# hukaixuan19970627/yolov5_obb

Hardware: AMD Instinct MI355X
Metric: val.py img/s (hot path: non_max_suppression_obb, bs16) + NMS ms/img @100k cand, DOTAv1.5 1024^2, 1/2/4/8 GPU (higher is better)
Workload: dtype f16; 1 GPU; DOTAv1.5 1024^2 bs16 (BASELINE metric; configs[1] thresholds): yolov5 OBB head output (16,64512,201) fp16, 4 distinct tensors rotated (cold: 1.66 GB working set) -> non_max_suppression_obb (conf .25, iou .45, multi_label, max_det 1500), val.py --task speed hot path = dt[2] of val.py; global_batch=16, anchors_per_image=64512, nc=16, detections_per_batch=3734, parallelism=dp1 (images sharded, no data-path collective)

## Files before the change

### include/obb_hip.h

```cpp
#ifndef OBB_HIP_H
#define OBB_HIP_H

#include <stddef.h>
#include <stdint.h>

#ifdef __cplusplus
extern "C" {
#endif

#define OBB_OK 0
#define OBB_ERR_BAD_ARG (-1)
#define OBB_ERR_WORKSPACE (-2)
#define OBB_ERR_LAUNCH (-3)
#define OBB_ERR_INTERNAL (-4)
#define OBB_ERR_NO_DEVICE (-5)

#define OBB_DTYPE_F32 0
#define OBB_DTYPE_F16 1
#define OBB_DTYPE_BF16 3

#define OBB_NMS_DROP_SMALL 1

const char* obb_version(void);
int obb_device_info(int* cu_count, int* wave_size, char* arch_name, int arch_name_len);
int obb_nms_set_max_grid(int max_workgroups);

#define OBB_PROF_STAGES 8
int obb_profile_enable(int on);
int obb_profile_collect(double* ms_sum_host, int64_t* count_host, int n_stages);



size_t obb_nms_workspace_bytes(int64_t n, int64_t nseg, int kind);

int obb_nms_rotated_f32(const float* dets5, const float* scores, int64_t n, float iou_thr, int flags, int64_t max_keep,
                        int64_t* keep_out, int64_t* num_keep, void* ws, size_t ws_bytes, void* stream);

int obb_nms_rotated_f64(const double* dets5, const double* scores, int64_t n, float iou_thr, int flags, int64_t max_keep,
                        int64_t* keep_out, int64_t* num_keep, void* ws, size_t ws_bytes, void* stream);

int obb_nms_poly_f32(const float* polys, int64_t row_stride, int64_t n, float iou_thr, int64_t max_keep, int64_t* keep_out,
                     int64_t* num_keep, void* ws, size_t ws_bytes, void* stream);

int obb_merge_nms_poly_f64(const double* dets9, int64_t n, const int32_t* order, const int32_t* seg_off, int64_t nseg,
// ... 197 lines not shown
```

### yolov5_obb_amd/_lib.py

```python
import ctypes as C
import os
import threading

import torch

_HERE = os.path.dirname(os.path.abspath(__file__))
LIB_PATH = os.environ.get("OBB_HIP_LIB") or os.path.join(_HERE, "libobb_hip.so")

OBB_OK = 0
OBB_NMS_DROP_SMALL = 1
_ERR = {-1: "bad argument", -2: "workspace missing or too small", -3: "kernel launch failed",
        -4: "internal error", -5: "no usable HIP device"}

_lib = None
_lock = threading.RLock()

_vp, _i64, _i32, _f32, _sz = C.c_void_p, C.c_int64, C.c_int, C.c_float, C.c_size_t

SIGNATURES = {
    "obb_version": (C.c_char_p, []),
    "obb_device_info": (_i32, [C.POINTER(_i32), C.POINTER(_i32), C.c_char_p, _i32]),
    "obb_nms_set_max_grid": (_i32, [_i32]),
    "obb_profile_enable": (_i32, [_i32]),
    "obb_profile_collect": (_i32, [_vp, _vp, _i32]),
    "obb_nms_workspace_bytes": (_sz, [_i64, _i64, _i32]),
    "obb_nms_rotated_f32": (_i32, [_vp, _vp, _i64, _f32, _i32, _i64, _vp, _vp, _vp, _sz, _vp]),
    "obb_nms_rotated_f64": (_i32, [_vp, _vp, _i64, _f32, _i32, _i64, _vp, _vp, _vp, _sz, _vp]),
    "obb_nms_poly_f32": (_i32, [_vp, _i64, _i64, _f32, _i64, _vp, _vp, _vp, _sz, _vp]),
    "obb_merge_nms_poly_f64": (_i32, [_vp, _i64, _vp, _vp, _i64, C.c_double, _vp, _vp, _vp, _sz, _vp]),
    "obb_merge_nms_poly_all_f64": (_i32, [_vp, _i64, _vp, _vp, _i64, C.c_double, _vp, _vp, _vp, _sz, _vp]),
    "obb_merge_nms_hbb_f64": (_i32, [_vp, _i64, _i64, _vp, _vp, _i64, C.c_double, _vp, _vp, _vp, _sz, _vp]),
    "obb_task1_parse_tiles": (_i64, [_vp, _i64, _i64, _vp, _vp, _vp, _vp, _vp, _vp]),
    "obb_task1_format_rows": (_i64, [_vp, _vp, _vp, _vp, _vp, _i64, _vp, _i64]),
    "obb_task1_parse_dets": (_i64, [_vp, _i64, _i64, _vp, _vp, _vp, _vp]),
    "obb_task1_parse_gt": (_i64, [_vp, _i64, _i64, _vp, _vp, _vp, _vp]),
    "obb_eval_best_gt_f64": (_i32, [_vp, _vp, _i64, _vp, _vp, _i64, _vp, _vp, _vp]),
    "obb_eval_best_gt_hbb_f64": (_i32, [_vp, _i64, _vp, _i64, _vp, _vp, _i64, _vp, _vp, _vp]),
    "obb_nms_obb_workspace_bytes": (_sz, [_i64, _i64, _i64, _i32]),
    "obb_non_max_suppression_obb": (_i32, [_vp, _i32, _i64, _i64, _i64, _f32, _f32, _vp, _i32, _i32, _i32, _i64, _i64, _f32,
# ... 265 lines not shown
```

### yolov5_obb_amd/csrc/nms.hip

```cpp
#include <hip/hip_runtime.h>
#include <cstring>
#include <stdint.h>
#include <stdlib.h>
#include <stdio.h>
#include <string.h>
#include <hip/hip_fp16.h>
#include "launch_once.h"
#include "obb_device.h"
#include "nms_core.h"
#include "nms_mk.h"
#include "obb_hip.h"
#include "psrs_sort.h"
#include "nms_small.h"
#include "segsort.h"
#include "ws_layout.h"
#include "nms_plan.h"

namespace obb {

enum { PROF_DECODE = 0, PROF_SEGSORT, PROF_PREP, PROF_STEPS, PROF_GATHER, PROF_NMS_SORT, PROF_NMS_PREP, PROF_NMS_STEPS, PROF_N };
struct ProfState {
  int on = 0;
  static constexpr int kMax = 8192;
  hipEvent_t ev0[kMax], ev1[kMax];
// ... 957 lines not shown
}

int obb_profile_collect(double* ms_sum, int64_t* count, int n_stages) {
  for (int i = 0; i < n_stages; i++) { ms_sum[i] = 0.0; count[i] = 0; }
  for (int k = 0; k < g_prof.used; k++) {
    float ms = 0.f;
    if (hipEventSynchronize(g_prof.ev1[k]) != hipSuccess) return OBB_ERR_INTERNAL;
    if (hipEventElapsedTime(&ms, g_prof.ev0[k], g_prof.ev1[k]) != hipSuccess) return OBB_ERR_INTERNAL;
    const int id = g_prof.id[k];
    if (id < n_stages) { ms_sum[id] += ms; count[id]++; }
  }
  g_prof.used = 0;
  return OBB_OK;
}

int obb_nms_set_max_grid(int max_workgroups) {
  g_max_grid = max_workgroups > 0 ? max_workgroups : 0;
  return OBB_OK;
}

const char* obb_version(void) { return "obb_hip 0.2 (gfx950)"; }

int obb_device_info(int* cu_count, int* wave_size, char* arch_name, int arch_name_len) {
  int dev = 0;
  if (hipGetDevice(&dev) != hipSuccess) return OBB_ERR_NO_DEVICE;
  hipDeviceProp_t p;
  if (hipGetDeviceProperties(&p, dev) != hipSuccess) return OBB_ERR_NO_DEVICE;
  if (cu_count) *cu_count = p.multiProcessorCount;
  if (wave_size) *wave_size = p.warpSize;
  if (arch_name && arch_name_len > 0) { strncpy(arch_name, p.gcnArchName, arch_name_len - 1); arch_name[arch_name_len - 1] = 0; }
// ... 32 lines not shown
```

### yolov5_obb_amd/csrc/nms_plan.h

```cpp
#pragma once
#include <stddef.h>
#include <stdint.h>
#include <stdlib.h>

#include "nms_limits.h"
#include "ws_layout.h"

namespace obb {

enum FbWord {
  kFbSteps = 0,
  kFbKept = 1,
  kFbSlabs = 2,
  kFbEnqueued = 3,
  kFbTicksPersist = 4,
  kFbTicksMk = 5,
  kFbKeptPersist = 6,
  kFbKeptMk = 7,
  kFbWords = 8
};
struct FbSnapshot { int w[kFbWords]; };
static inline FbSnapshot fb_snapshot(const int* words) {
  FbSnapshot s;
  for (int i = 0; i < kFbWords; i++) s.w[i] = *(const volatile int*)(words + i);
  return s;
}

static inline int env_mk(const char* e) { return e ? atoi(e) : 2; }
static inline int env_mk_xlds(const char* e) { return (e && (e[0] == '0' || e[0] == '1')) ? e[0] - '0' : -1; }
static inline int env_small_helpers(const char* e) { const int v = (e && *e) ? atoi(e) : -1; return v > kSmallHelpMax ? kSmallHelpMax : v; }
static inline int env_self_sort(const char* e) { return (e && *e >= '0' && *e <= '2') ? *e - '0' : 2; }
static inline int env_mk_steps(const char* e) { return e ? atoi(e) : 0; }
static inline int env_mk_pend(const char* e) { const int v = e ? atoi(e) : 0; return (v > 0 && v < kMkPend1) ? v : kMkPend1; }
static inline int env_phase_prof(const char* e) { return (e && atoi(e)) ? 1 : 0; }
static inline int env_poly_strict(const char* e) { const int v = e ? atoi(e) : 0; return v == 1 ? 1 : (v >= 2 ? 0 : 3); }

struct NmsEnv {
  int mk;
  int mk_xlds;
  int small_helpers;
  int self_sort;
  int mk_steps;
  int mk_pend;
  int phase_prof;
  int quad_skip;
};
static inline NmsEnv nms_env() {
  static const NmsEnv process = [] {
    NmsEnv e{};
    e.mk_steps = env_mk_steps(getenv("OBB_NMS_MK_STEPS")); e.mk_pend = env_mk_pend(getenv("OBB_NMS_MK_PEND"));
    e.phase_prof = env_phase_prof(getenv("OBB_NMS_PHASE_PROF")); e.quad_skip = env_poly_strict(getenv("OBB_NMS_POLY_STRICT"));
    return e;
  }();
  NmsEnv e = process;
  e.mk = env_mk(getenv("OBB_NMS_MK")); e.mk_xlds = env_mk_xlds(getenv("OBB_NMS_MK_XLDS"));
  e.small_helpers = env_small_helpers(getenv("OBB_NMS_SMALL_HELPERS")); e.self_sort = env_self_sort(getenv("OBB_NMS_SELF_SORT"));
  return e;
}

static inline int nms_window(long long max_keep) {
  if (max_keep <= 0) return 0;
  long long w = 4 * max_keep;
  if (w < 8192) w = 8192;
  if (w > (1 << 30)) w = 1 << 30;
  return (int)((w + 63) / 64 * 64);
}
static inline int nms_grid(int64_t nseg, int64_t n_slots, int cap_first_, int cus) {
  int64_t nb = (n_slots + 511) / 512;
  {
    const int64_t per_seg = (n_slots + nseg - 1) / nseg;
    const int64_t c = per_seg < cap_first_ ? per_seg : cap_first_;
// ... 81 lines not shown
struct SmallHelpBlocks { int *work, *seg_np, *seg_ticket; unsigned long long *part_main, *part_help; };
static inline SmallHelpBlocks small_help_layout(WsCursor& w, int helpers, int64_t nseg, int64_t n_pos) {
  SmallHelpBlocks b;
  b.work = w.take<int>((size_t)helpers);
  b.seg_np = w.take<int>((size_t)nseg); b.seg_ticket = w.take<int>((size_t)nseg);
  b.part_main = w.take<unsigned long long>((size_t)n_pos * kSmallWords);
  b.part_help = w.take<unsigned long long>((size_t)helpers * kSmallMax * kSmallWords);
  return b;
}
static inline size_t small_help_bytes(int helpers, int64_t nseg, int64_t n_pos) {
  WsCursor w(nullptr);
  small_help_layout(w, helpers, nseg, n_pos);
  return w.total();
}

struct ObbPlanIn {
  int64_t bs, A;
  int nc, agnostic, multi_label;
  float iou_thres, max_wh;
  int64_t n_extra;
  int64_t cap_img;
  int64_t max_nms, max_det;
  int64_t expected_cand;
  int out_packed;
  int hw_cus, cus;
  long long ecap;
  size_t sort_tmp_bytes;
  size_t ps_scratch_bytes;
};
struct ObbPlan {
  int ncs;
  int class_ok;
  int multi_label;
  int64_t expected_cand, seg_hint;
  int small_hint;
  int lds_sort;
  int small_nms;
  int self_sort;
  int helpers;
  int fused_out;
  int rows_per_thread;
  int parts;
  int plan_nb, plan_chunk;
  int64_t max_seg;
  unsigned radix_mask;
  int psrs;
  unsigned gparts;
  int window;
  int zero_bar;
  int zero_alive;
};

static inline ObbPlan plan_nms_obb(const ObbPlanIn& in, const NmsEnv& env) {
  ObbPlan p{};
  const int64_t bs = in.bs, cap_img = in.cap_img;
  p.seg_hint = (in.expected_cand >> 32) & 0x1fffffff;
  p.small_hint = ((in.expected_cand >> 62) & 1) != 0;
  p.expected_cand = in.expected_cand & 0xffffffffll;
  p.ncs = in.agnostic ? 1 : in.nc;
  const int64_t nseg = bs * p.ncs;
  p.class_ok = (!in.agnostic && in.nc > 1 && in.A + in.n_extra < (1ll << 24) && in.iou_thres >= 0.f && in.max_wh > 0.f) ? 1 : 0;
  p.multi_label = (in.multi_label && in.nc > 1) ? 1 : 0;
  p.lds_sort = p.expected_cand > 0 && p.expected_cand <= kSortLdsHint;
  p.rows_per_thread = (bs * in.A >= 4LL * kDecThreads * 480) ? 4 : (bs * in.A >= 2LL * kDecThreads * 480) ? 2 : 1;
  p.max_seg = (in.max_nms > 0 && in.max_nms < cap_img) ? in.max_nms : cap_img;
// ... 16 lines not shown
    if (!p.self_sort) p.parts = (p.class_ok && p.ncs >= 8) ? 4 : 1;
  } else {
    int tb = 0;
    while ((1ll << tb) < in.A * in.nc + in.n_extra + 1) tb++;
    unsigned mask = 0xF0u;
    for (int d = 0; d < 4; d++) if (tb > d * 8) mask |= 1u << d;
    if (p.class_ok) mask = 0xFFu;
    p.radix_mask = mask;
    p.psrs = bs == 1 && cap_img <= kPsMaxN && in.sort_tmp_bytes >= in.ps_scratch_bytes;
  }
  p.fused_out = p.small_nms && !in.out_packed;
  if (!p.fused_out)
    p.gparts = p.expected_cand <= 2048 ? 1u : (unsigned)((p.expected_cand + 1023) / 1024 > 16 ? 16 : (p.expected_cand + 1023) / 1024);
  p.zero_bar = (!p.small_nms || !p.fused_out) ? 1 : 0;
  p.zero_alive = (p.lds_sort && !p.self_sort) ? 1 : 0;
  return p;
}

}
```

### yolov5_obb_amd/csrc/nms_small.h

```cpp
#pragma once
#include "nms_limits.h"

namespace obb {

#ifdef OBB_SMALL_TRACE
__device__ unsigned long long g_small_trace[2048 * 16];
__device__ unsigned long long g_small_trace_tail[2048 * 4];
__device__ unsigned long long g_small_trace2[2048 * 8];
#define STRACE(kind, ...) do { if (threadIdx.x == 0 && blockIdx.x < 2048) { const unsigned long long v_[] = {__VA_ARGS__}; unsigned long long* o_ = g_small_trace + blockIdx.x * 16; o_[0] = (kind); for (int z_ = 0; z_ < (int)(sizeof(v_) / 8) && z_ < 15; z_++) o_[1 + z_] = v_[z_]; } } while (0)
#endif
constexpr int kSmallThreads = 512;
constexpr int kSmallWaves = kSmallThreads / 64;

struct SmallArgs {
  const float4* rec;
  const u64* alive;
  const int* seg_begin;
  const int* seg_end;
  int* keep_cnt;
  int64_t* keep_out;
  int* too_big;
  float thr;
  int max_keep;
  const unsigned long long* keys_sorted;
// ... 6 lines not shown
  int helpers;
  const int* help_cnt;
  const int* work;
  const int* seg_np;
  int* seg_ticket;
  u64* part_main;
  u64* part_help;
  const unsigned long long* keys_in;
  const float4* cand;
  const int* cnt;
  const int* tiny;
  long long cap_img, max_nms, A;
  int nc;
  float class_offset;
  int* seg_max;
};
struct SmallFromSort { static constexpr bool kSelf = false; };
constexpr int kSmallClipWaves = 4;
constexpr int kSmallSplit1 = 128;
__host__ __device__ __forceinline__ int small_parts(int n) {
  return n <= kSmallSplit1 ? 1 : (n <= 192 ? 2 : (n <= 256 ? 4 : (n <= 320 ? 6 : 8)));
}
struct SmallNoTail {
  struct Args {};
  static __device__ __forceinline__ void run(const SmallArgs&, const Args&, unsigned char*, int) {}
};

template <class G>
__device__ __attribute__((noinline)) int small_quick(const float4* ra, const float4* rb, float thr) {
  return G::classify_quick(ra, rb, thr, true);
}
// ... 24 lines not shown
  uint32_t q0[128], q1[128], q2[128];
};

template <class G, class FRONT>
__device__ __forceinline__ int small_segment(const SmallArgs& a, unsigned char* s_raw) {
  __shared__ int s_next, s_nkept, s_qcnt[kSmallWaves], s_qhead[kSmallWaves], s_qcnt2[kSmallWaves], s_last;
  __shared__ uint32_t s_kept[kSmallMax];
  __shared__ unsigned long long s_pk[kSmallMax];
  __shared__ uint32_t s_pv[kSmallMax];
  float4* s_rec = reinterpret_cast<float4*>(s_raw);
  u64* s_mask = reinterpret_cast<u64*>(s_rec + (size_t)kSmallMax * G::RECQ);
  u64* s_alive = s_mask + (size_t)kSmallMax * kSmallWords;
  SmallWave<G>* s_wave = reinterpret_cast<SmallWave<G>*>(s_alive + 8);
  const int tid = threadIdx.x, lane = tid & 63, wv = tid >> 6;
  int seg = (int)blockIdx.x - a.helpers, part = 0, np = 1, hbase = 0;
  if (seg < 0) {
    const int h = (int)blockIdx.x;
    if (h >= *a.help_cnt) {
#ifdef OBB_SMALL_TRACE
      STRACE(1ull, (unsigned long long)wall_clock64());
#endif
      return -1;
    }
    const int e = a.work[h];
    if (e < 0) return -1;
    seg = e & 0xffffff; part = e >> 24;
  }
  if (a.helpers > 0) { const int v = a.seg_np[seg]; if ((v & 255) > 1) { np = v & 255; hbase = v >> 8; } }
#ifdef OBB_SMALL_TRACE
  unsigned long long tt[8]; int ti_ = 0, nd0 = 0, nd1 = 0, nd2 = 0, nit = 0;
  unsigned long long acc_d0 = 0, acc_d1 = 0, acc_d2 = 0, acc_draw = 0, acc_l0 = 0, acc_l1 = 0, acc_l2 = 0;
#define SSTAMP() do { tt[ti_++] = wall_clock64(); } while (0)
#else
#define SSTAMP() do {} while (0)
#endif
  SSTAMP();
  int sb, n, md_self = 0;
  if constexpr (FRONT::kSelf) {
    const int r = FRONT::template load<G>(a, seg, reinterpret_cast<float4*>(s_raw),
                                          reinterpret_cast<u64*>(reinterpret_cast<float4*>(s_raw) + (size_t)kSmallMax * G::RECQ), s_pk, s_pv, &s_next);
    n = r & 0xffff; md_self = r >> 16;
    sb = (int)((long long)(seg / a.ncs) * a.cap_img) + (seg % a.ncs) * kSmallMax;
    if (n <= 0 || n > kSmallMax) {
      if (tid == 0) { stg_agent(a.keep_cnt + seg, 0); if (n > kSmallMax) atomicMax(a.too_big, n); }
      return seg;
    }
  } else {
    sb = a.seg_begin[seg]; n = a.seg_end[seg] - sb;
    if (n <= 0) return part == 0 ? seg : -1;
    if (n > kSmallMax) { if (tid == 0 && part == 0) atomicMax(a.too_big, n); return part == 0 ? seg : -1; }
  }
  const bool pub = a.pub_key != nullptr;
  if constexpr (!FRONT::kSelf) {
    for (int t = tid; t < n * G::RECQ; t += kSmallThreads) s_rec[t] = a.rec[(size_t)sb * G::RECQ + t];
    for (int t = tid; t < n * kSmallWords; t += kSmallThreads) s_mask[t] = 0ull;
    if (pub)
      for (int t = tid; t < n; t += kSmallThreads) { s_pk[t] = a.keys_sorted[(size_t)sb + t]; s_pv[t] = a.vals_sorted[(size_t)sb + t]; }
    if (tid < kSmallWords) {
      const int w0 = (sb >> 6) + tid, sh = sb & 63;
      u64 v = a.alive[w0] >> sh;
// ... 171 lines not shown
          Q.head = (Q.head + took) & 127; Q.count -= took;
        }
        if (busy) {
          if (stage == 0) { Q1.push(res == 3, e); Q2.push(res == 2, e); }
          else if (stage == 1) Q2.push(res == 2, e);
          wave_sync();
        }
        __syncthreads();
      }
    }
  }
  SSTAMP();
  __syncthreads();
  if (np > 1) {
    auto part_buf = [&](int p) -> u64* {
      return p == 0 ? a.part_main + (size_t)sb * kSmallWords : a.part_help + (size_t)(hbase + p - 1) * kSmallMax * kSmallWords;
    };
    u64* mine = part_buf(part);
    for (int t = tid; t < n * kSmallWords; t += kSmallThreads) stg_agent(mine + t, s_mask[t]);
    asm volatile("s_waitcnt vmcnt(0)" ::: "memory");
    __syncthreads();
    if (tid == 0) s_last = __hip_atomic_fetch_add(a.seg_ticket + seg, 1, __ATOMIC_RELAXED, __HIP_MEMORY_SCOPE_AGENT) == np - 1 ? 1 : 0;
    __syncthreads();
    if (!s_last) {
#ifdef OBB_SMALL_TRACE
      STRACE(2ull, (unsigned long long)seg | ((unsigned long long)part << 24) | ((unsigned long long)np << 28), (unsigned long long)n, 0ull, tt[0], tt[1], tt[2], tt[3], (unsigned long long)wall_clock64(), 0ull, 0ull, (unsigned long long)nit, (unsigned long long)nd0, (unsigned long long)nd1, (unsigned long long)nd2);
#endif
      return -1;
    }
    for (int p = 0; p < np; p++) {
      if (p == part) continue;
      const u64* src = part_buf(p);
      for (int t = tid; t < n * kSmallWords; t += kSmallThreads) { const u64 v = ldg_agent(src + t); if (v) s_mask[t] |= v; }
    }
    __syncthreads();
  }
  SSTAMP();
// ... 62 lines not shown
```

### yolov5_obb_amd/csrc/nmsobb_impl.h

```cpp
#pragma once
#include "dtype_device.h"
#include "obb_device.h"
#include "segsort.h"
#include "nms_plan.h"

namespace obb {

struct ClassMask { unsigned long long w[4]; int all; };

template <typename T> __device__ __forceinline__ float mul_in_dtype(float a, float b);
template <> __device__ __forceinline__ float mul_in_dtype<float>(float a, float b) { return a * b; }
template <> __device__ __forceinline__ float mul_in_dtype<__half>(float a, float b) { return __half2float(__float2half_rn(a * b)); }
template <> __device__ __forceinline__ float mul_in_dtype<bf16_t>(float a, float b) { return round_to_dtype<bf16_t>(a * b); }
template <typename T> __device__ __forceinline__ float thr_in_dtype(float t);
template <> __device__ __forceinline__ float thr_in_dtype<float>(float t) { return t; }
template <> __device__ __forceinline__ float thr_in_dtype<__half>(float t) { return __half2float(__float2half_rn(t)); }
template <> __device__ __forceinline__ float thr_in_dtype<bf16_t>(float t) { return round_to_dtype<bf16_t>(t); }

__device__ __forceinline__ unsigned long long argmax_key(float v, int i) {
  const uint32_t b = __float_as_uint(v + 0.0f);
  const uint32_t m = (v != v) ? 0xFFFFFFFFu : (b & 0x80000000u) ? ~b : (b | 0x80000000u);
  return ((unsigned long long)m << 32) | (unsigned long long)(0xFFFFFFFFu - (uint32_t)i);
}
template <int CTRL>
// ... 35 lines not shown
  int no, nc, bs;
  float conf_thres;
  int multi_label;
  int rows_per_thread;
  ClassMask cm;
  long long cap_img;
  float4* cand;
  unsigned long long* keys;
  uint32_t* vals;
  int* cnt;
  int* tiny;
  float win_lo, win_hi;
  int* z_ticket; int n_ticket;
  uint4* z_bar16; long long n_bar16;
  uint4* z_alive16; long long n_alive16;
};

constexpr int kImgSmall = 1, kImgWide = 2, kImgChecked = 4, kImgCross = 8;
__host__ __device__ __forceinline__ bool img_single_list(int t) {
  return (t & kImgWide) || ((t & kImgSmall) && (!(t & kImgChecked) || (t & kImgCross)));
}
__device__ __forceinline__ int cand_flags(float x, float l, float s, float win_lo, float win_hi) {
  const float mn = min_nan(l, s);
  const float rr = sqrtf(l * l + s * s) * 0.501f + 0.5f;
  int f = (mn >= 0.001f && mn < 1.0f) ? kImgSmall : 0;
  if (!(x - rr > win_lo && x + rr < win_hi)) f |= kImgWide;
  return f;
}

__device__ __forceinline__ bool class_allowed(const ClassMask& cm, int c) {
// ... 52 lines not shown
  const T* csl = base + 5 + nc;
#pragma unroll
  for (int k = 0; k < kDecCslRegs; k++) r.csl[k] = ld_as_float<T>((k * 16 + l16 < 180) ? csl + k * 16 + l16 : base);
#pragma unroll
  for (int g = 0; g < kDecClsRegs; g++) r.cls[g] = ld_as_float<T>((g * 16 + l16 < nc) ? base + 5 + g * 16 + l16 : base);
#pragma unroll
  for (int k = 0; k < 4; k++) r.box[k] = ld_as_float<T>(base + k);
  return r;
}

template <typename T>
__global__ __launch_bounds__(kDecThreads) void k_decode(DecodeArgs a) {
  __shared__ float4 s_c0[kDecWaves][kDecStage], s_c1[kDecWaves][kDecStage];
  __shared__ unsigned long long s_key[kDecWaves][kDecStage];
  __shared__ int s_cnt[kDecWaves], s_base, s_n;
  __shared__ uint32_t s_row[kDecThreads * kDecMaxG];
  __shared__ float s_obj[kDecThreads * kDecMaxG];

  const T* pred = (const T*)a.pred;
  const int tid = threadIdx.x, lane = tid & 63, wv = tid >> 6;
  const int b = blockIdx.y;
  const int G = a.rows_per_thread;
  const float thr = thr_in_dtype<T>(a.conf_thres);
  const T* img = pred + (size_t)b * a.A * a.no;
  float4* cand = a.cand + (size_t)b * a.cap_img * 2;
  unsigned long long* keys = a.keys + (size_t)b * a.cap_img;
  uint32_t* vals = a.vals + (size_t)b * a.cap_img;
  float4* c0s = s_c0[wv]; float4* c1s = s_c1[wv]; unsigned long long* kys = s_key[wv];
  int staged = 0;
  int flags_seen = 0;
  if (tid == 0) s_n = 0;
  DTRACE_DECL();

  auto write_out = [&](long long base, int count) {
    for (int i = lane; i < count; i += 64) {
      const long long slot = base + i;
      if (slot < a.cap_img) {
        cand[slot * 2] = c0s[i];
        cand[slot * 2 + 1] = c1s[i];
        keys[slot] = kys[i];
        vals[slot] = (uint32_t)slot;
      }
    }
  };
  auto flush_wave = [&]() {
    int base = 0;
// ... 42 lines not shown

  const int l16 = lane & 15, sub = lane >> 4;
  const int ncg = (a.nc + 15) >> 4;
  struct RowOut { float bx, by, bl, bs_, theta; int bflags; long long rw; };
  auto stage = [&](const RowOut& o, bool p, float conf, int c) {
    const unsigned long long pb = __ballot(p);
    const int np = __popcll(pb);
    if (np == 0) return;
    if (staged + np > kDecStage) flush_wave();
    if (p) {
      const int i = staged + __popcll(pb & lanemask_lt());
      c0s[i] = make_float4(o.bx, o.by, o.bl, o.bs_);
      c1s[i] = make_float4(o.theta, conf, (float)c, 0.f);
      kys[i] = ((unsigned long long)score_desc_key(conf) << 32) | (unsigned long long)(uint32_t)(o.rw * a.nc + c);
      flags_seen |= o.bflags;
    }
    staged += np;
    DTRACE_ADD(11, np);
  };
  auto row_out = [&](float bx, float by, float bl, float bs_, unsigned long long tk, uint32_t row) {
    float tv; int ti;
    argmax_unkey(row_max_u64(tk), tv, ti);
    RowOut o;
    o.bx = bx; o.by = by; o.bl = bl; o.bs_ = bs_;
    o.theta = ((float)(ti - 90) / 180.0f) * 3.141592f;
    o.bflags = cand_flags(bx, bl, bs_, a.win_lo, a.win_hi);
    o.rw = (long long)row;
    return o;
  };
  auto stage_best = [&](const RowOut& o, bool valid, unsigned long long bestk) {
// ... 41 lines not shown
    if (fl && lane == 0) atomicOr(&a.tiny[b], fl);
  }
  DTRACE_WAVE(6, 7);
  if (lane == 0) s_cnt[wv] = staged;
  __syncthreads();
  if (threadIdx.x == 0) {
    int tot = 0;
    for (int w = 0; w < kDecWaves; w++) tot += s_cnt[w];
    s_base = tot ? atomicAdd(&a.cnt[b * kCntPad], tot) : 0;
  }
  __syncthreads();
  DTRACE_T0(8);
  int base = s_base;
  for (int w = 0; w < wv; w++) base += s_cnt[w];
  write_out(base, staged);
  DTRACE_END(n_rows);
}

__global__ void k_append_extra(const float* __restrict__ extra8, int m, long long A, int nc, DecodeArgs a) {
  int i = blockIdx.x * blockDim.x + threadIdx.x;
  if (i >= m) return;
  const float* e = extra8 + (size_t)i * 8;
  const int b = (int)e[0];
  if (b < 0 || b >= a.bs) return;
  if (!(e[6] > a.conf_thres) || !class_allowed(a.cm, (int)e[7])) return;
  const int slot = atomicAdd(&a.cnt[b * kCntPad], 1);
  { const int fl = cand_flags(e[1], e[3], e[4], a.win_lo, a.win_hi); if (fl) atomicOr(&a.tiny[b], fl); }
  if (slot >= a.cap_img) return;
  const size_t g = (size_t)b * a.cap_img + slot;
  a.cand[g * 2] = make_float4(e[1], e[2], e[3], e[4]);
// ... 531 lines not shown
    o[0] = c0.x; o[1] = c0.y; o[2] = c0.z; o[3] = c0.w; o[4] = c1.x; o[5] = c1.y; o[6] = c1.z;
  }
}

struct SmallSelfSort {
  static constexpr bool kSelf = true;
  static __device__ __forceinline__ int image_mode(long long c, int tf, long long cap_img, long long max_nms, int& n, int& e) {
    const bool over_cap = c > cap_img;
    if (over_cap) c = cap_img;
    if (c > kSortLdsMax) c = 0;
    const bool over_nms = max_nms > 0 && c > max_nms;
    e = (int)(over_nms ? max_nms : c);
    n = (int)c;
    return (!over_cap && !img_single_list(tf) && !over_nms) ? 1 : 0;
  }
  template <class G>
  static __device__ __forceinline__ int load(const SmallArgs& a, int seg, float4* s_rec, u64* s_mask, unsigned long long* s_pk,
                                                       uint32_t* s_pv, int* s_n) {
    const int tid = threadIdx.x, lane = tid & 63;
    const int g = seg / a.ncs, c = seg - g * a.ncs;
    constexpr int KPT = 8;
    const size_t b0 = (size_t)g * (size_t)a.cap_img;
    const int spec = a.cap_img < (long long)KPT * kSmallThreads ? (int)a.cap_img : KPT * kSmallThreads;
    unsigned long long k[KPT];
#pragma unroll
    for (int u = 0; u < KPT; u++) { const int i = u * kSmallThreads + tid; k[u] = i < spec ? a.keys_in[b0 + i] : 0ull; }
    int n, e;
    const int m = image_mode(a.cnt[g * kCntPad], a.tiny[g], a.cap_img, a.max_nms, n, e);
    if (n == 0 || (m == 0 && c != 0)) return m << 16;
    u64* s_alive = s_mask + (size_t)kSmallMax * kSmallWords;
    unsigned long long* st_key = reinterpret_cast<unsigned long long*>(s_mask);
    uint32_t* st_slot = reinterpret_cast<uint32_t*>(st_key + kSmallMax);
    if (tid == 0) *s_n = 0;
    if (tid < 8) s_alive[tid] = 0ull;
    __syncthreads();
    const uint32_t nc = (uint32_t)a.nc, lim = (uint32_t)((unsigned long long)a.A * nc);
    for (int i0 = 0; i0 < n; i0 += KPT * kSmallThreads) {
      if (i0 > 0) {
#pragma unroll
        for (int u = 0; u < KPT; u++) { const int i = i0 + u * kSmallThreads + tid; k[u] = i < n ? a.keys_in[b0 + i] : 0ull; }
      }
#pragma unroll
      for (int u = 0; u < KPT; u++) {
// ... 283 lines not shown
  size_t total;
};

static inline int64_t round_cap(int64_t cap_img) { return (cap_img + 63) / 64 * 64; }

static ObbCarve obb_carve(void* base, int64_t bs, int64_t cap_img, int64_t ncs) {
  cap_img = round_cap(cap_img);
  ObbCarve cv{};
  WsCursor w(base);
  const size_t n = (size_t)bs * cap_img;
  cv.cand = w.take<float4>(n * 2);
  cv.keys_a = w.take<unsigned long long>(n); cv.keys_b = w.take<unsigned long long>(n);
  cv.vals_a = w.take<uint32_t>(n); cv.vals_b = w.take<uint32_t>(n);
  cv.cnt = w.take<int>(bs * kCntPad); cv.sort_begin = w.take<int>(bs); cv.sort_end = w.take<int>(bs);
  cv.img_end = w.take<int>(bs); cv.mode = w.take<int>(bs); cv.tiny = w.take<int>(bs);
  cv.ticket = w.take<int>(16 + (size_t)(bs + 1));
  cv.seg_size = w.take<int>((size_t)bs * 256);
  cv.srs_hist = w.take<uint32_t>((size_t)bs * ((size_t)(cap_img + kSrsTile - 1) / kSrsTile) * 256);
  cv.keep = w.take<int64_t>(n);
  w.nest([&](void* b) { return (cv.nms = carve(b, (int64_t)n, bs * ncs, RotGeom::RECQ, cap_max(bs * ncs))).total; });
  cv.total = w.total();
  return cv;
}

struct HeadFront;
struct HeadFrontTta;
static int launch_decode_head(const HeadFront& h, const DecodeArgs& d, int dtype, hipStream_t st);
static int launch_decode_head_tta(const HeadFrontTta& h, const DecodeArgs& d, int dtype, hipStream_t st);

static int run_nms_obb(const void* pred, const void* objcol, int dtype, int64_t bs, int64_t A, int64_t no, float conf_thres, float iou_thres,
                       const int32_t* classes_host, int n_classes, int agnostic, int multi_label, int64_t max_det, int64_t max_nms,
// ... 1 lines not shown
                       int out_packed, int64_t* out_count, int64_t* status, void* ws, size_t ws_bytes, hipStream_t st, void* state = nullptr,
                       size_t state_bytes = 0, const HeadFront* head = nullptr, const HeadFrontTta* tta = nullptr) {
  const int nc = (int)(no - 5 - 180);
  if (bs < 1 || A < 1 || nc < 1 || nc > 256 || max_det < 1 || cap_img < 1 || (!pred && !head && !tta) || !out || !out_count || !status)
    return OBB_ERR_BAD_ARG;
  if (A * nc + n_extra > 0xffffffffLL || bs * cap_img > 0x7fffffffLL) return OBB_ERR_BAD_ARG;
  if (!dtype_known(dtype)) return OBB_ERR_BAD_ARG;
  cap_img = round_cap(cap_img);
  ObbCarve cv = obb_carve(ws, bs, cap_img, agnostic ? 1 : nc);
  if (!ws_ok(ws, ws_bytes, cv.total)) return OBB_ERR_WORKSPACE;
  ObbPlanIn pin{};
  pin.bs = bs; pin.A = A; pin.nc = nc; pin.agnostic = agnostic; pin.multi_label = multi_label; pin.iou_thres = iou_thres; pin.max_wh = max_wh;
  pin.n_extra = n_extra; pin.cap_img = cap_img; pin.max_nms = max_nms; pin.max_det = max_det; pin.expected_cand = expected_cand;
  pin.out_packed = out_packed; pin.hw_cus = hw_cu_count(); pin.cus = cu_count(); pin.ecap = cv.nms.ecap;
  pin.sort_tmp_bytes = cv.nms.sort_tmp_bytes; pin.ps_scratch_bytes = ps_scratch_bytes();
  const ObbPlan plan = plan_nms_obb(pin, nms_env());
  const int ncs = plan.ncs, class_ok = plan.class_ok, helpers = plan.helpers;
  int rc = OBB_OK;
  const bool kept = state != nullptr;
  if (kept) {
    if (!ws_ok(state, state_bytes, obb_state_bytes(bs))) return OBB_ERR_WORKSPACE;
    cv.cnt = (int*)state;
    cv.tiny = cv.cnt + bs * kCntPad;
  }

  DecodeArgs d;
  d.pred = pred; d.objcol = objcol; d.A = A; d.no = (int)no; d.nc = nc; d.bs = (int)bs; d.conf_thres = conf_thres;
  d.multi_label = plan.multi_label;
  d.cm.all = (classes_host == nullptr || n_classes <= 0) ? 1 : 0;
  for (int i = 0; i < 4; i++) d.cm.w[i] = 0ull;
  for (int i = 0; i < n_classes && classes_host; i++) {
    int c = classes_host[i];
    if (c >= 0 && c < 256) d.cm.w[c >> 6] |= 1ull << (c & 63);
  }
  d.cap_img = cap_img; d.cand = cv.cand; d.keys = cv.keys_a; d.vals = cv.vals_a; d.cnt = cv.cnt; d.tiny = cv.tiny;
  d.win_lo = -0.35f * max_wh; d.win_hi = 0.6f * max_wh;

  d.z_ticket = nullptr; d.n_ticket = 0; d.z_bar16 = nullptr; d.n_bar16 = 0; d.z_alive16 = nullptr; d.n_alive16 = 0;
  {
    Carve& nv0 = cv.nms;
    const long long alive16 = plan.zero_alive ? (long long)((((size_t)bs * cap_img) >> 6) + 8 + 1) / 2 : 0ll;
    const long long bar16 = plan.zero_bar ? (long long)(nv0.bar_bytes / 16) : 0ll;
    if (kept) {
      d.z_ticket = cv.ticket; d.n_ticket = (int)(16 + bs + 1);
      d.z_bar16 = bar16 ? reinterpret_cast<uint4*>(nv0.bar) : nullptr; d.n_bar16 = bar16;
      d.z_alive16 = alive16 ? reinterpret_cast<uint4*>(nv0.alive) : nullptr; d.n_alive16 = alive16;
    } else {
      k_reset_state<<<256, 256, 0, st>>>(cv.cnt, (int)(bs * kCntPad), cv.tiny, (int)bs, status, cv.ticket, (int)(16 + bs + 1),
                                         reinterpret_cast<uint4*>(nv0.bar), bar16, reinterpret_cast<uint4*>(nv0.alive), alive16);
    }
  }
  d.rows_per_thread = plan.rows_per_thread;
  dim3 gd((unsigned)((A + kDecThreads * d.rows_per_thread - 1) / (kDecThreads * d.rows_per_thread)), (unsigned)bs);
  {
    ProfScope ps(PROF_DECODE, st);
    if (head || tta) {
      rc = head ? launch_decode_head(*head, d, dtype, st) : launch_decode_head_tta(*tta, d, dtype, st);
      if (rc) return rc;
    } else OBB_DISPATCH_DTYPE(dtype, T, k_decode<T><<<gd, kDecThreads, 0, st>>>(d));
  }
  if (n_extra > 0 && extra8) k_append_extra<<<(unsigned)((n_extra + 255) / 256), 256, 0, st>>>(extra8, (int)n_extra, A, nc, d);
  if (plan.small_hint && class_ok)
    k_tiny_cross<<<dim3(kTinyParts, (unsigned)bs), 256, 0, st>>>(cv.cand, cv.keys_a, cv.cnt, cap_img, max_wh, iou_thres, cv.tiny);
// ... 64 lines not shown
    static OncePerDevice attr;
    const size_t lds = small_lds_bytes<RotGeom>();
    if (const int attr_dev = attr.need(); attr_dev != OncePerDevice::kDone) {
      if (hipFuncSetAttribute((const void*)k_nms_small<RotGeom, SmallNoTail>, hipFuncAttributeMaxDynamicSharedMemorySize, (int)lds) != hipSuccess ||
          hipFuncSetAttribute((const void*)k_nms_small<RotGeom, SmallGather>, hipFuncAttributeMaxDynamicSharedMemorySize, (int)lds) != hipSuccess ||
          hipFuncSetAttribute((const void*)k_nms_small<RotGeom, SmallGather, SmallSelfSort>, hipFuncAttributeMaxDynamicSharedMemorySize, (int)lds) != hipSuccess)
        return OBB_ERR_LAUNCH;
      attr.mark(attr_dev);
    }
    SmallArgs sa{};
    sa.rec = nv.rec; sa.alive = nv.alive; sa.seg_begin = nv.seg_begin; sa.seg_end = nv.seg_end; sa.keep_cnt = nv.keep_cnt;
    sa.keep_out = cv.keep; sa.too_big = cv.ticket + 8; sa.thr = iou_thres; sa.max_keep = (int)max_det;
    sa.ncs = ncs; sa.mode = cv.mode;
    sa.helpers = helpers; sa.help_cnt = cv.ticket + 12; sa.work = hb.work; sa.seg_np = hb.seg_np; sa.seg_ticket = hb.seg_ticket;
    sa.part_main = hb.part_main; sa.part_help = hb.part_help;
    const unsigned gsmall = (unsigned)(bs * ncs + helpers);
    if (plan.fused_out) {
      sa.keys_sorted = cv.keys_b; sa.vals_sorted = cv.vals_b; sa.pub_key = cv.keys_a; sa.pub_val = cv.vals_a; sa.n_pos = bs * cap_img;
      SmallGather::Args ga{};
      ga.cand = cv.cand; ga.cnt = cv.cnt; ga.tiny = cv.tiny; ga.info = cv.ticket; ga.ticket = cv.ticket + 16;
      ga.out = out; ga.out_count = out_count; ga.status = status; ga.cap_img = cap_img; ga.max_det = max_det; ga.bs = (int)bs;
      ga.clean_cnt = kept ? cv.cnt : nullptr; ga.clean_tiny = kept ? cv.tiny : nullptr;
      if (plan.self_sort) {
        sa.pub_key = cv.keys_b; sa.pub_val = cv.vals_b; sa.keys_sorted = nullptr; sa.vals_sorted = nullptr;
        sa.keys_in = cv.keys_a; sa.cand = cv.cand; sa.cnt = cv.cnt; sa.tiny = cv.tiny; sa.cap_img = cap_img; sa.max_nms = max_nms; sa.A = A; sa.nc = nc;
        sa.class_offset = max_wh; sa.seg_max = cv.ticket + 4;
        k_nms_small<RotGeom, SmallGather, SmallSelfSort><<<gsmall, kSmallThreads, lds, st>>>(sa, ga);
      } else
      k_nms_small<RotGeom, SmallGather><<<gsmall, kSmallThreads, lds, st>>>(sa, ga);
    } else {
      k_nms_small<RotGeom, SmallNoTail><<<gsmall, kSmallThreads, lds, st>>>(sa, SmallNoTail::Args{});
    }
  } else {
    ProfScope ps(PROF_STEPS, st);
    rc = nms_steps(0, a, nv, bs * ncs, bs * max_seg, st, kNmsBarZeroed | ((plan.lds_sort && plan.plan_nb > 0) ? kNmsPlanned : 0));
    if (rc) return rc;
  }
  if (!plan.fused_out) {
    ProfScope ps(PROF_GATHER, st);
    k_gather_out<<<dim3((unsigned)bs, plan.gparts), 256, 0, st>>>(cv.cand, cv.vals_b, cv.keys_b, cv.keep, nv.seg_begin, nv.keep_cnt, cv.mode, ncs, max_det,
                                              out, out_count, cv.cnt, cap_img, status, nv.abort_flag, out_packed, cv.ticket, cv.tiny,
// ... 7 lines not shown
```

Measured before the change: 160,900 img/s.

## Split oversized per-class NMS segments across helper blocks using decode-time class histograms

The decode kernel now optionally counts candidates per class in shared memory and writes per-workgroup histograms to global memory. In the self-sorting small-NMS kernel, extra helper blocks read these histograms to estimate segment sizes. They then pick a size threshold that fits a helper budget, and each takes one part of a large segment's suppression work, with results merged through a ticket. The goal is to cut tail latency from a few long class segments. The cost is extra histogram atomics in decode, an added block-wide scan, workspace carving and more ticket zeroing. It is gated on free CUs beyond the segment count, so on a full-size device it may fall back to no sharing.

```diff
diff --git a/include/obb_hip.h b/include/obb_hip.h
--- a/include/obb_hip.h
+++ b/include/obb_hip.h
@@ -28,6 +28,7 @@
 #define OBB_PROF_STAGES 8
 int obb_profile_enable(int on);
 int obb_profile_collect(double* ms_sum_host, int64_t* count_host, int n_stages);
+int obb_nms_small_share_parts(int64_t* parts_host);
 
 
 
diff --git a/yolov5_obb_amd/_lib.py b/yolov5_obb_amd/_lib.py
--- a/yolov5_obb_amd/_lib.py
+++ b/yolov5_obb_amd/_lib.py
@@ -23,6 +23,7 @@
     "obb_nms_set_max_grid": (_i32, [_i32]),
     "obb_profile_enable": (_i32, [_i32]),
     "obb_profile_collect": (_i32, [_vp, _vp, _i32]),
+    "obb_nms_small_share_parts": (_i32, [_vp]),
     "obb_nms_workspace_bytes": (_sz, [_i64, _i64, _i32]),
     "obb_nms_rotated_f32": (_i32, [_vp, _vp, _i64, _f32, _i32, _i64, _vp, _vp, _vp, _sz, _vp]),
     "obb_nms_rotated_f64": (_i32, [_vp, _vp, _i64, _f32, _i32, _i64, _vp, _vp, _vp, _sz, _vp]),
diff --git a/yolov5_obb_amd/csrc/nms.hip b/yolov5_obb_amd/csrc/nms.hip
--- a/yolov5_obb_amd/csrc/nms.hip
+++ b/yolov5_obb_amd/csrc/nms.hip
@@ -995,6 +995,14 @@
   return OBB_OK;
 }
 
+int obb_nms_small_share_parts(int64_t* parts_host) {
+  if (!parts_host) return OBB_ERR_BAD_ARG;
+  unsigned long long v = 0ull;
+  if (hipMemcpyFromSymbol(&v, HIP_SYMBOL(obb::g_small_share_parts), sizeof(v)) != hipSuccess) return OBB_ERR_INTERNAL;
+  *parts_host = (int64_t)v;
+  return OBB_OK;
+}
+
 int obb_nms_set_max_grid(int max_workgroups) {
   g_max_grid = max_workgroups > 0 ? max_workgroups : 0;
   return OBB_OK;
diff --git a/yolov5_obb_amd/csrc/nms_plan.h b/yolov5_obb_amd/csrc/nms_plan.h
--- a/yolov5_obb_amd/csrc/nms_plan.h
+++ b/yolov5_obb_amd/csrc/nms_plan.h
@@ -4,6 +4,7 @@
 #include <stdlib.h>
 
 #include "nms_limits.h"
+#include "small_share.h"
 #include "ws_layout.h"
 
 namespace obb {
@@ -30,6 +31,11 @@
 static inline int env_mk_xlds(const char* e) { return (e && (e[0] == '0' || e[0] == '1')) ? e[0] - '0' : -1; }
 static inline int env_small_helpers(const char* e) { const int v = (e && *e) ? atoi(e) : -1; return v > kSmallHelpMax ? kSmallHelpMax : v; }
 static inline int env_self_sort(const char* e) { return (e && *e >= '0' && *e <= '2') ? *e - '0' : 2; }
+static inline int env_small_share(const char* e) {
+  if (!(e && *e)) return 0;
+  const int v = atoi(e);
+  return v <= 0 ? -1 : (v > kSmallHelpMax ? kSmallHelpMax : v);
+}
 static inline int env_mk_steps(const char* e) { return e ? atoi(e) : 0; }
 static inline int env_mk_pend(const char* e) { const int v = e ? atoi(e) : 0; return (v > 0 && v < kMkPend1) ? v : kMkPend1; }
 static inline int env_phase_prof(const char* e) { return (e && atoi(e)) ? 1 : 0; }
@@ -44,6 +50,7 @@
   int mk_pend;
   int phase_prof;
   int quad_skip;
+  int small_share;
 };
 static inline NmsEnv nms_env() {
   static const NmsEnv process = [] {
@@ -55,6 +62,7 @@
   NmsEnv e = process;
   e.mk = env_mk(getenv("OBB_NMS_MK")); e.mk_xlds = env_mk_xlds(getenv("OBB_NMS_MK_XLDS"));
   e.small_helpers = env_small_helpers(getenv("OBB_NMS_SMALL_HELPERS")); e.self_sort = env_self_sort(getenv("OBB_NMS_SELF_SORT"));
+  e.small_share = env_small_share(getenv("OBB_NMS_SMALL_SHARE"));
   return e;
 }
 
@@ -166,6 +174,19 @@
   return w.total();
 }
 
+struct SmallShareBlocks { int* part_hist; unsigned long long* part_buf; };
+static inline SmallShareBlocks small_share_layout(WsCursor& w, int share, int64_t nseg, int hist_lg) {
+  SmallShareBlocks b;
+  b.part_hist = w.take<int>((size_t)nseg << hist_lg);
+  b.part_buf = w.take<unsigned long long>((size_t)2 * share * kSmallMax * kSmallWords);
+  return b;
+}
+static inline size_t small_share_bytes(int share, int64_t nseg, int hist_lg) {
+  WsCursor w(nullptr);
+  small_share_layout(w, share, nseg, hist_lg);
+  return w.total();
+}
+
 struct ObbPlanIn {
   int64_t bs, A;
   int nc, agnostic, multi_label;
@@ -179,6 +200,7 @@
   long long ecap;
   size_t sort_tmp_bytes;
   size_t ps_scratch_bytes;
+  int front;
 };
 struct ObbPlan {
   int ncs;
@@ -201,6 +223,7 @@
   int window;
   int zero_bar;
   int zero_alive;
+  int share, share_budget, dec_wgs, hist_lg;
 };
 
 static inline ObbPlan plan_nms_obb(const ObbPlanIn& in, const NmsEnv& env) {
@@ -247,6 +270,16 @@
     p.gparts = p.expected_cand <= 2048 ? 1u : (unsigned)((p.expected_cand + 1023) / 1024 > 16 ? 16 : (p.expected_cand + 1023) / 1024);
   p.zero_bar = (!p.small_nms || !p.fused_out) ? 1 : 0;
   p.zero_alive = (p.lds_sort && !p.self_sort) ? 1 : 0;
+  p.dec_wgs = (int)((in.A + (int64_t)kDecThreads * p.rows_per_thread - 1) / ((int64_t)kDecThreads * p.rows_per_thread));
+  p.hist_lg = share_hist_lg(p.dec_wgs);
+  if (p.self_sort && p.fused_out && in.front == 0 && in.n_extra == 0 && env.small_share >= 0 && (nseg << p.hist_lg) <= kShareMaxHist) {
+    const int64_t free_cus = (int64_t)in.hw_cus - nseg;
+    if (env.small_share > 0) { p.share = env.small_share; p.share_budget = p.share; }
+    else if (free_cus > 0) { p.share = (int)(free_cus > kSmallHelpMax ? kSmallHelpMax : free_cus); p.share_budget = p.share; }
+    else { p.share = kShareFullPool; p.share_budget = kShareFullBudget; }
+    const size_t have = (size_t)(nseg < (int64_t)in.cus ? nseg : (int64_t)in.cus) * (size_t)in.ecap * 4;
+    if (small_share_bytes(p.share, nseg, p.hist_lg) > have) { p.share = 0; p.share_budget = 0; }
+  }
   return p;
 }
 
diff --git a/yolov5_obb_amd/csrc/nms_small.h b/yolov5_obb_amd/csrc/nms_small.h
--- a/yolov5_obb_amd/csrc/nms_small.h
+++ b/yolov5_obb_amd/csrc/nms_small.h
@@ -1,7 +1,10 @@
 #pragma once
 #include "nms_limits.h"
+#include "small_share.h"
 
 namespace obb {
+
+__device__ unsigned long long g_small_share_parts;
 
 #ifdef OBB_SMALL_TRACE
 __device__ unsigned long long g_small_trace[2048 * 16];
@@ -44,7 +47,58 @@
   int nc;
   float class_offset;
   int* seg_max;
+  const int* part_hist;
+  int dec_wgs, hist_lg, share_budget;
 };
+__device__ __attribute__((noinline)) int small_share_eval(int my_n, int nseg, int B, int query_seg, int query_slot) {
+  __shared__ unsigned long long s_tot[kSmallWaves];
+  __shared__ int s_res;
+  const int tid = threadIdx.x, lane = tid & 63, wv = tid >> 6;
+  unsigned long long v = 0ull;
+  if (tid < nseg) {
+#pragma unroll
+    for (int r = 0; r < kShareRungs; r++) v |= (unsigned long long)share_extra(my_n, share_rung(r)) << (12 * r);
+  }
+  unsigned long long inc = v;
+#pragma unroll
+  for (int d = 1; d < 64; d <<= 1) { const unsigned long long t = __shfl_up(inc, d); if (lane >= d) inc += t; }
+  if (lane == 63) s_tot[wv] = inc;
+  if (tid == 0) s_res = -1;
+  __syncthreads();
+  unsigned long long tot = 0ull;
+#pragma unroll
+  for (int w = 0; w < kSmallWaves; w++) { const unsigned long long t = s_tot[w]; tot += t; if (w < wv) inc += t; }
+  int need[kShareRungs];
+#pragma unroll
+  for (int r = 0; r < kShareRungs; r++) need[r] = (int)((tot >> (12 * r)) & 0xfffull);
+  const int sh = 12 * share_pick(need, B);
+  const int ex = (int)((v >> sh) & 0xfffull), base = (int)((inc >> sh) & 0xfffull) - ex;
+  const bool shared = share_fits(base, ex, B);
+  if (query_seg >= 0) { if (tid == query_seg) s_res = shared ? ((ex + 1) | (base << 8)) : 1; }
+  else if (shared && query_slot >= base && query_slot < base + ex) s_res = tid | ((query_slot - base + 1) << 12) | ((ex + 1) << 16) | (base << 20);
+  __syncthreads();
+  return s_res;
+}
+__device__ __attribute__((noinline)) int small_share_sizes(uint4 h0, uint4 h1, uint4 h2, uint4 h3, int dec_wgs, int hist_lg, int nseg) {
+  __shared__ int s_size[kShareMaxSeg];
+  const int tid = threadIdx.x;
+  if (tid < kShareMaxSeg) s_size[tid] = 0;
+  __syncthreads();
+  const int seg = tid >> (hist_lg - 4), w0 = (tid * 16) & ((1 << hist_lg) - 1);
+  if (seg < nseg) {
+    const uint32_t v[16] = {h0.x, h0.y, h0.z, h0.w, h1.x, h1.y, h1.z, h1.w, h2.x, h2.y, h2.z, h2.w, h3.x, h3.y, h3.z, h3.w};
+    int sum = 0;
+#pragma unroll
+    for (int u = 0; u < 16; u++) sum += w0 + u < dec_wgs ? (int)v[u] : 0;
+    if (sum) atomicAdd(&s_size[seg], sum);
+  }
+  __syncthreads();
+  return tid < nseg ? s_size[tid] : 0;
+}
+static_assert(kShareMaxHist == 16 * kSmallThreads && kShareMaxSeg == kShareMaxHist / 16, "small_share_sizes: sixteen words per thread");
+static_assert(kShareMaxSeg <= kSmallThreads && 3 * kShareMaxSeg < 4096 && kShareMaxParts <= 4 && kShareRungs * 12 <= 64 && kSmallHelpMax <= 256,
+              "small_share_eval: one thread per segment, 12-bit slot sums, slots below 2^8");
+
 struct SmallFromSort { static constexpr bool kSelf = false; };
 constexpr int kSmallClipWaves = 4;
 constexpr int kSmallSplit1 = 128;
@@ -99,6 +153,23 @@
   SmallWave<G>* s_wave = reinterpret_cast<SmallWave<G>*>(s_alive + 8);
   const int tid = threadIdx.x, lane = tid & 63, wv = tid >> 6;
   int seg = (int)blockIdx.x - a.helpers, part = 0, np = 1, hbase = 0;
+  const bool sharing = FRONT::kSelf && a.part_hist != nullptr;
+  const int nseg_l = (int)gridDim.x - a.helpers;
+  uint4 hv[4];
+  if constexpr (FRONT::kSelf) {
+    if (seg < 0) {
+      FRONT::hist_request(a, nseg_l, hv);
+      const int hint = small_share_sizes(hv[0], hv[1], hv[2], hv[3], a.dec_wgs, a.hist_lg, nseg_l);
+      const int e = small_share_eval(hint, nseg_l, a.share_budget, -1, (int)blockIdx.x);
+      if (e < 0) {
+#ifdef OBB_SMALL_TRACE
+        STRACE(1ull, (unsigned long long)wall_clock64());
+#endif
+        return -1;
+      }
+      seg = e & 0xfff; part = (e >> 12) & 15; np = (e >> 16) & 15; hbase = e >> 20;
+    }
+  } else {
   if (seg < 0) {
     const int h = (int)blockIdx.x;
     if (h >= *a.help_cnt) {
@@ -112,6 +183,7 @@
     seg = e & 0xffffff; part = e >> 24;
   }
   if (a.helpers > 0) { const int v = a.seg_np[seg]; if ((v & 255) > 1) { np = v & 255; hbase = v >> 8; } }
+  }
 #ifdef OBB_SMALL_TRACE
   unsigned long long tt[8]; int ti_ = 0, nd0 = 0, nd1 = 0, nd2 = 0, nit = 0;
   unsigned long long acc_d0 = 0, acc_d1 = 0, acc_d2 = 0, acc_draw = 0, acc_l0 = 0, acc_l1 = 0, acc_l2 = 0;
@@ -123,12 +195,19 @@
   int sb, n, md_self = 0;
   if constexpr (FRONT::kSelf) {
     const int r = FRONT::template load<G>(a, seg, reinterpret_cast<float4*>(s_raw),
-                                          reinterpret_cast<u64*>(reinterpret_cast<float4*>(s_raw) + (size_t)kSmallMax * G::RECQ), s_pk, s_pv, &s_next);
+                                          reinterpret_cast<u64*>(reinterpret_cast<float4*>(s_raw) + (size_t)kSmallMax * G::RECQ), s_pk, s_pv, &s_next,
+                                          hv, sharing && part == 0, nseg_l);
     n = r & 0xffff; md_self = r >> 16;
     sb = (int)((long long)(seg / a.ncs) * a.cap_img) + (seg % a.ncs) * kSmallMax;
     if (n <= 0 || n > kSmallMax) {
+      if (part != 0) return -1;
       if (tid == 0) { stg_agent(a.keep_cnt + seg, 0); if (n > kSmallMax) atomicMax(a.too_big, n); }
       return seg;
+    }
+    if (sharing && part == 0) {
+      const int hint = small_share_sizes(hv[0], hv[1], hv[2], hv[3], a.dec_wgs, a.hist_lg, nseg_l);
+      const int e = small_share_eval(hint, nseg_l, a.share_budget, seg, -1);
+      np = e & 255; hbase = e >> 8;
     }
   } else {
     sb = a.seg_begin[seg]; n = a.seg_end[seg] - sb;
@@ -330,6 +409,7 @@
   __syncthreads();
   if (np > 1) {
     auto part_buf = [&](int p) -> u64* {
+      if constexpr (FRONT::kSelf) return a.part_help + (size_t)(p == 0 ? a.helpers + hbase : hbase + p - 1) * kSmallMax * kSmallWords;
       return p == 0 ? a.part_main + (size_t)sb * kSmallWords : a.part_help + (size_t)(hbase + p - 1) * kSmallMax * kSmallWords;
     };
     u64* mine = part_buf(part);
@@ -337,6 +417,7 @@
     asm volatile("s_waitcnt vmcnt(0)" ::: "memory");
     __syncthreads();
     if (tid == 0) s_last = __hip_atomic_fetch_add(a.seg_ticket + seg, 1, __ATOMIC_RELAXED, __HIP_MEMORY_SCOPE_AGENT) == np - 1 ? 1 : 0;
+    if (FRONT::kSelf && tid == 0 && part > 0) atomicAdd(&g_small_share_parts, 1ull);
     __syncthreads();
     if (!s_last) {
 #ifdef OBB_SMALL_TRACE
diff --git a/yolov5_obb_amd/csrc/nmsobb_impl.h b/yolov5_obb_amd/csrc/nmsobb_impl.h
--- a/yolov5_obb_amd/csrc/nmsobb_impl.h
+++ b/yolov5_obb_amd/csrc/nmsobb_impl.h
@@ -73,6 +73,7 @@
   int* z_ticket; int n_ticket;
   uint4* z_bar16; long long n_bar16;
   uint4* z_alive16; long long n_alive16;
+  int* part_hist; int hist_lg;
 };
 
 constexpr int kImgSmall = 1, kImgWide = 2, kImgChecked = 4, kImgCross = 8;
@@ -155,6 +156,7 @@
   __shared__ float4 s_c0[kDecWaves][kDecStage], s_c1[kDecWaves][kDecStage];
   __shared__ unsigned long long s_key[kDecWaves][kDecStage];
   __shared__ int s_cnt[kDecWaves], s_base, s_n;
+  __shared__ int s_hist[256];
   __shared__ uint32_t s_row[kDecThreads * kDecMaxG];
   __shared__ float s_obj[kDecThreads * kDecMaxG];
 
@@ -171,6 +173,8 @@
   int staged = 0;
   int flags_seen = 0;
   if (tid == 0) s_n = 0;
+  const bool hist = a.part_hist != nullptr;
+  if (hist && tid < 256) s_hist[tid] = 0;
   DTRACE_DECL();
 
   auto write_out = [&](long long base, int count) {
@@ -243,6 +247,7 @@
       c1s[i] = make_float4(o.theta, conf, (float)c, 0.f);
       kys[i] = ((unsigned long long)score_desc_key(conf) << 32) | (unsigned long long)(uint32_t)(o.rw * a.nc + c);
       flags_seen |= o.bflags;
+      if (hist) atomicAdd(&s_hist[c], 1);
     }
     staged += np;
     DTRACE_ADD(11, np);
@@ -314,6 +319,7 @@
   int base = s_base;
   for (int w = 0; w < wv; w++) base += s_cnt[w];
   write_out(base, staged);
+  if (hist && tid < a.nc) a.part_hist[(((size_t)b * a.nc + tid) << a.hist_lg) + blockIdx.x] = s_hist[tid];
   DTRACE_END(n_rows);
 }
 
@@ -875,9 +881,15 @@
     n = (int)c;
     return (!over_cap && !img_single_list(tf) && !over_nms) ? 1 : 0;
   }
+  static __device__ __forceinline__ void hist_request(const SmallArgs& a, int nseg, uint4 (&hv)[4]) {
+    const int t = (int)threadIdx.x, seg = t >> (a.hist_lg - 4);
+    const uint4* p = reinterpret_cast<const uint4*>(a.part_hist) + (seg < nseg ? (size_t)t * 4 : 0);
+#pragma unroll
+    for (int u = 0; u < 4; u++) hv[u] = p[u];
+  }
   template <class G>
   static __device__ __forceinline__ int load(const SmallArgs& a, int seg, float4* s_rec, u64* s_mask, unsigned long long* s_pk,
-                                                       uint32_t* s_pv, int* s_n) {
+                                                       uint32_t* s_pv, int* s_n, uint4 (&hv)[4], bool want_hist, int nseg) {
     const int tid = threadIdx.x, lane = tid & 63;
     const int g = seg / a.ncs, c = seg - g * a.ncs;
     constexpr int KPT = 8;
@@ -887,7 +899,9 @@
 #pragma unroll
     for (int u = 0; u < KPT; u++) { const int i = u * kSmallThreads + tid; k[u] = i < spec ? a.keys_in[b0 + i] : 0ull; }
     int n, e;
-    const int m = image_mode(a.cnt[g * kCntPad], a.tiny[g], a.cap_img, a.max_nms, n, e);
+    const int cnt_g = a.cnt[g * kCntPad], tiny_g = a.tiny[g];
+    if (want_hist) hist_request(a, nseg, hv);
+    const int m = image_mode(cnt_g, tiny_g, a.cap_img, a.max_nms, n, e);
     if (n == 0 || (m == 0 && c != 0)) return m << 16;
     u64* s_alive = s_mask + (size_t)kSmallMax * kSmallWords;
     unsigned long long* st_key = reinterpret_cast<unsigned long long*>(s_mask);
@@ -1201,7 +1215,7 @@
   cv.vals_a = w.take<uint32_t>(n); cv.vals_b = w.take<uint32_t>(n);
   cv.cnt = w.take<int>(bs * kCntPad); cv.sort_begin = w.take<int>(bs); cv.sort_end = w.take<int>(bs);
   cv.img_end = w.take<int>(bs); cv.mode = w.take<int>(bs); cv.tiny = w.take<int>(bs);
-  cv.ticket = w.take<int>(16 + (size_t)(bs + 1));
+  cv.ticket = w.take<int>(16 + (size_t)(bs + 1) + (size_t)(bs * ncs));
   cv.seg_size = w.take<int>((size_t)bs * 256);
   cv.srs_hist = w.take<uint32_t>((size_t)bs * ((size_t)(cap_img + kSrsTile - 1) / kSrsTile) * 256);
   cv.keep = w.take<int64_t>(n);
@@ -1233,8 +1247,12 @@
   pin.n_extra = n_extra; pin.cap_img = cap_img; pin.max_nms = max_nms; pin.max_det = max_det; pin.expected_cand = expected_cand;
   pin.out_packed = out_packed; pin.hw_cus = hw_cu_count(); pin.cus = cu_count(); pin.ecap = cv.nms.ecap;
   pin.sort_tmp_bytes = cv.nms.sort_tmp_bytes; pin.ps_scratch_bytes = ps_scratch_bytes();
+  pin.front = (head || tta) ? 1 : 0;
   const ObbPlan plan = plan_nms_obb(pin, nms_env());
-  const int ncs = plan.ncs, class_ok = plan.class_ok, helpers = plan.helpers;
+  const int ncs = plan.ncs, class_ok = plan.class_ok, helpers = plan.helpers, share = plan.share;
+  SmallShareBlocks sb{};
+  if (share > 0) { WsCursor w(cv.nms.edges); sb = small_share_layout(w, share, bs * ncs, plan.hist_lg); }
+  const int n_ticket = (int)(16 + bs + 1 + (share > 0 ? bs * ncs : 0));
   int rc = OBB_OK;
   const bool kept = state != nullptr;
   if (kept) {
@@ -1255,17 +1273,18 @@
   d.cap_img = cap_img; d.cand = cv.cand; d.keys = cv.keys_a; d.vals = cv.vals_a; d.cnt = cv.cnt; d.tiny = cv.tiny;
   d.win_lo = -0.35f * max_wh; d.win_hi = 0.6f * max_wh;
 
+  d.part_hist = share > 0 ? sb.part_hist : nullptr; d.hist_lg = plan.hist_lg;
   d.z_ticket = nullptr; d.n_ticket = 0; d.z_bar16 = nullptr; d.n_bar16 = 0; d.z_alive16 = nullptr; d.n_alive16 = 0;
   {
     Carve& nv0 = cv.nms;
     const long long alive16 = plan.zero_alive ? (long long)((((size_t)bs * cap_img) >> 6) + 8 + 1) / 2 : 0ll;
     const long long bar16 = plan.zero_bar ? (long long)(nv0.bar_bytes / 16) : 0ll;
     if (kept) {
-      d.z_ticket = cv.ticket; d.n_ticket = (int)(16 + bs + 1);
+      d.z_ticket = cv.ticket; d.n_ticket = n_ticket;
       d.z_bar16 = bar16 ? reinterpret_cast<uint4*>(nv0.bar) : nullptr; d.n_bar16 = bar16;
       d.z_alive16 = alive16 ? reinterpret_cast<uint4*>(nv0.alive) : nullptr; d.n_alive16 = alive16;
     } else {
-      k_reset_state<<<256, 256, 0, st>>>(cv.cnt, (int)(bs * kCntPad), cv.tiny, (int)bs, status, cv.ticket, (int)(16 + bs + 1),
+      k_reset_state<<<256, 256, 0, st>>>(cv.cnt, (int)(bs * kCntPad), cv.tiny, (int)bs, status, cv.ticket, n_ticket,
                                          reinterpret_cast<uint4*>(nv0.bar), bar16, reinterpret_cast<uint4*>(nv0.alive), alive16);
     }
   }
@@ -1360,7 +1379,7 @@
     sa.ncs = ncs; sa.mode = cv.mode;
     sa.helpers = helpers; sa.help_cnt = cv.ticket + 12; sa.work = hb.work; sa.seg_np = hb.seg_np; sa.seg_ticket = hb.seg_ticket;
     sa.part_main = hb.part_main; sa.part_help = hb.part_help;
-    const unsigned gsmall = (unsigned)(bs * ncs + helpers);
+    unsigned gsmall = (unsigned)(bs * ncs + helpers);
     if (plan.fused_out) {
       sa.keys_sorted = cv.keys_b; sa.vals_sorted = cv.vals_b; sa.pub_key = cv.keys_a; sa.pub_val = cv.vals_a; sa.n_pos = bs * cap_img;
       SmallGather::Args ga{};
@@ -1371,6 +1390,11 @@
         sa.pub_key = cv.keys_b; sa.pub_val = cv.vals_b; sa.keys_sorted = nullptr; sa.vals_sorted = nullptr;
         sa.keys_in = cv.keys_a; sa.cand = cv.cand; sa.cnt = cv.cnt; sa.tiny = cv.tiny; sa.cap_img = cap_img; sa.max_nms = max_nms; sa.A = A; sa.nc = nc;
         sa.class_offset = max_wh; sa.seg_max = cv.ticket + 4;
+        if (share > 0) {
+          sa.helpers = share; sa.share_budget = plan.share_budget; sa.part_hist = sb.part_hist; sa.dec_wgs = plan.dec_wgs; sa.hist_lg = plan.hist_lg;
+          sa.part_help = sb.part_buf; sa.seg_ticket = cv.ticket + 16 + bs + 1;
+          gsmall = (unsigned)(bs * ncs + share);
+        }
         k_nms_small<RotGeom, SmallGather, SmallSelfSort><<<gsmall, kSmallThreads, lds, st>>>(sa, ga);
       } else
       k_nms_small<RotGeom, SmallGather><<<gsmall, kSmallThreads, lds, st>>>(sa, ga);
diff --git a/yolov5_obb_amd/csrc/small_share.h b/yolov5_obb_amd/csrc/small_share.h
--- /dev/null
+++ b/yolov5_obb_amd/csrc/small_share.h
@@ -0,0 +1,53 @@
+#pragma once
+
+#if defined(__HIPCC__) || defined(__CUDACC__)
+#define OBB_SHARE_HD __host__ __device__
+#else
+#define OBB_SHARE_HD
+#endif
+
+namespace obb {
+
+constexpr int kShareRungs = 5;
+constexpr int kShareMaxSeg = 512;
+constexpr int kShareMaxHist = 8192;
+OBB_SHARE_HD inline int share_hist_lg(int dec_wgs) { int lg = 4; while ((1 << lg) < dec_wgs && lg < 30) lg++; return lg; }
+constexpr int kShareMaxParts = 4;
+constexpr int kShareFullPool = 0;
+constexpr int kShareFullBudget = 0;
+
+OBB_SHARE_HD inline int share_rung(int r) { return r <= 0 ? 128 : (r == 1 ? 160 : (r == 2 ? 192 : (r == 3 ? 224 : 256))); }
+OBB_SHARE_HD inline int share_parts_of(int n) { return n <= 176 ? 2 : (n <= 240 ? 3 : kShareMaxParts); }
+OBB_SHARE_HD inline int share_extra(int n, int T) { return n > T ? share_parts_of(n) - 1 : 0; }
+OBB_SHARE_HD inline int share_pick(const int* need, int B) {
+  for (int r = 0; r < kShareRungs; r++)
+    if (need[r] <= B) return r;
+  return kShareRungs - 1;
+}
+OBB_SHARE_HD inline bool share_fits(int base, int extra, int B) { return extra > 0 && base + extra <= B; }
+
+OBB_SHARE_HD inline int small_share_schedule(const int* n, int nseg, int H, int B, int* np, int* first, int* slot) {
+  if (H < 0) H = 0;
+  if (B > H) B = H;
+  if (B < 0) B = 0;
+  int need[kShareRungs];
+  for (int r = 0; r < kShareRungs; r++) {
+    need[r] = 0;
+    for (int s = 0; s < nseg; s++) need[r] += share_extra(n[s], share_rung(r));
+  }
+  const int r = share_pick(need, B), T = share_rung(r);
+  for (int h = 0; h < H; h++) slot[h] = -1;
+  int base = 0;
+  for (int s = 0; s < nseg; s++) {
+    const int ex = share_extra(n[s], T);
+    np[s] = 1; first[s] = -1;
+    if (share_fits(base, ex, B)) {
+      np[s] = ex + 1; first[s] = base;
+      for (int p = 1; p <= ex; p++) slot[base + p - 1] = s | (p << 16);
+    }
+    base += ex;
+  }
+  return r;
+}
+
+}
```

Result: slower. 158,900 img/s (-1.2%).
